# Dzh-16/FLASH-Viterbi

Hardware: AMD Instinct MI355X
Metric: trellis_cells_per_sec (higher is better)
Workload: dtype f32 scores (+f64 add per cell, rounded to f32 as the reference does)

## Files before the change

### flash_viterbi_amd/csrc/fv_context.hip

```cpp
#include "fv_internal.h"
#include "flashvit_testing.h"

namespace {

template <typename F>
void parallel_rows(int rows, F &&fn)
{
    unsigned hw = std::thread::hardware_concurrency();
    int nt = (int)std::min<unsigned>(hw ? hw : 4, 16);
    if (rows < 256) nt = 1;
    if (nt <= 1) { fn(0, rows); return; }
    std::vector<std::thread> th;
    int per = (rows + nt - 1) / nt;
    for (int t = 0; t < nt; ++t) {
        int a = t * per, b = std::min(rows, a + per);
        if (a >= b) break;
        th.emplace_back([=, &fn] { fn(a, b); });
    }
    for (auto &x : th) x.join();
}

}

namespace fvi {
// ... 922 lines not shown
        if (int rc = fvi::launch_stage_emissions(ctx, dev_scores, dtype, ld, T, ctx->EMap.p, ctx->emis_P, ctx->E32.p, ctx->E64.p, ctx->d_emflags.p)) return fvi::drained(ctx, rc);
    FV_HIP(hipEventRecord(e1, ctx->stream));
    FV_HIP(hipStreamSynchronize(ctx->stream));
    float ms = 0.0f;
    FV_HIP(hipEventElapsedTime(&ms, e0, e1));
    *ms_out = ms / (float)reps;
    ctx->stats.device_bytes = (long long)fvi::device_bytes(ctx);
    return FV_OK;
}

extern "C" int fv_test_flat_poison(fv_ctx *ctx, int t)
{
    if (!ctx || t < -1) return FV_ERR_ARG;
    FV_NO_STREAM(ctx);
    ctx->flat_poison = t;
    return FV_OK;
}

extern "C" int fv_set_option(fv_ctx *ctx, int key, long long value)
{
    if (!ctx) return FV_ERR_ARG;
    FV_NO_STREAM(ctx);
    if (ctx->group && ctx->group_rank == 0) {
        for (int r = fvi::group_size(ctx) - 1; r >= 1; --r) {
            const int rc = fv_set_option(fvi::group_member(ctx, r), key, value);
            if (rc) return rc;
        }
    }
    switch (key) {
    case FV_OPT_KERNEL:
        if ((value < FV_KERNEL_AUTO || value > FV_KERNEL_U16_REFINE) && value != FV_KERNEL_CSR_F64) return FV_ERR_ARG;
        ctx->opt_kernel = (int)value; return FV_OK;
    case FV_OPT_MAX_BATCH:
        if (value < 1 || value > fvk::MAX_BATCH) return FV_ERR_ARG;
        ctx->opt_max_batch = (int)value; return FV_OK;
    case FV_OPT_PROFILE:
        ctx->opt_profile = value ? 1 : 0; return FV_OK;
    case FV_OPT_FLAT_GENERATIONS:
        if (value < 0 || value > 2) return FV_ERR_ARG;
        ctx->opt_flat = (int)value; return FV_OK;
    case FV_OPT_ROW_CODES:
        if (value < 0 || value > 4) return FV_ERR_ARG;
        ctx->opt_row_codes = (int)value; return FV_OK;
    case FV_OPT_SEL_MARGIN:
        if (value < 0 || value > 100000) return FV_ERR_ARG;
        ctx->opt_sel_margin = (float)value * 1e-3f; return FV_OK;
    case FV_OPT_SPARSE_BEAM:
        if (value != 0 && value != 1) return FV_ERR_ARG;
        ctx->opt_sparse_beam = (int)value; return FV_OK;
    case FV_OPT_DEBUG:
#ifndef FV_TIMING_BUILD
        if (value & FV_DEBUG_TIMING_ONLY) { ctx->detail = "FV_OPT_DEBUG: result-changing timing switches need the timing build"; return FV_ERR_ARG; }
#endif
        if (value < 0 || value >= (1ll << 32) || (value & ((1ll << 27) | (1ll << 30)))) return FV_ERR_ARG;
        ctx->opt_csr_mem = (int)((value >> 31) & 1);
        ctx->opt_debug = (int)(value & 0x3fffffff); return FV_OK;
    default: return FV_ERR_ARG;
    }
}

extern "C" long long fv_checkpoint_memory_bytes(int K, int T, int step)
{
    if (step <= 0) step = (int)std::floor(std::sqrt(1.0 * T));
    const long long nck = (T + step - 1) / step;
    const long long last = T - (nck - 1) * step;
    const long long tsub = nck > 1 && step + 1 > last ? step + 1 : last;
    return 4LL * K + 4LL * K * nck + 4LL * K + 4LL * (T / step + 1) + 8LL * K * tsub;
}

extern "C" int fv_last_stats(const fv_ctx *ctx, fv_stats *out)
{
    if (!ctx || !out) return FV_ERR_ARG;
    *out = ctx->stats;
    return FV_OK;
}

extern "C" const char *fv_last_error_detail(const fv_ctx *ctx) { return ctx ? ctx->detail.c_str() : ""; }

extern "C" const char *fv_strerror(int rc)
{
    switch (rc) {
    case FV_OK: return "ok";
    case FV_WARN_BEAM_MISS: return "beam miss: path holds -1 entries, as the reference prints";
    case FV_ERR_ARG: return "bad argument";
    case FV_ERR_NOMEM: return "out of memory";
    case FV_ERR_NO_PRED: return "decoded entry has no finite predecessor";
    case FV_ERR_DEVICE: return "HIP error";
    case FV_ERR_STATE: return "call out of order (no model / no communicator)";
    case FV_ERR_UNSUPPORTED: return "size or option not supported by this build";
    case FV_ERR_COMM: return "RCCL error";
    default: return "unknown flashvit error";
    }
}

extern "C" long long fv_reference_memory_bytes(int K, int T, int n_split, int beam_width)
{
    const long long N = n_split;
    const long long pool = ((40 + 48 + 8 * N + 12 + 7) / 8) * 8;
    long long mem = 0, tmp;
    const bool nway = N > 2 && T >= 2 * N;
    if (beam_width <= 0) {
        if (nway) mem = 4 * (N - 1) + 2LL * K * 4 + 2 * (N - 1) * (long long)K * 4;
        tmp = N * (2LL * K * 4 + 2LL * K * 4);
    } else {
        if (nway) mem = 4 * (N - 1) + 2 * (N - 1) * (long long)(beam_width + 1) * 12;
        tmp = N * (2LL * (beam_width + 1) * 12);
    }
    if (tmp > mem) mem = tmp;
// ... 3 lines not shown
```

### flash_viterbi_amd/csrc/fv_full.hip

```cpp
#include "fv_internal.h"
#include "fv_kernels.hip.inc"
#include "flashvit_testing.h"

namespace {

int pick_kernel(const fv_ctx *ctx)
{
    if (ctx->opt_kernel == FV_KERNEL_F64_STREAM) return FV_KERNEL_F64_STREAM;
    if (!ctx->view.logs_nonpositive) return FV_KERNEL_F64_STREAM;
    if (ctx->opt_kernel == FV_KERNEL_F16_REFINE || ctx->opt_kernel == FV_KERNEL_F32_REFINE ||
        ctx->opt_kernel == FV_KERNEL_Q16_REFINE || ctx->opt_kernel == FV_KERNEL_U16_REFINE)
        return ctx->opt_kernel;
    if (ctx->opt_kernel == FV_KERNEL_SPARSE_Q16) return ctx->SPdata.p ? FV_KERNEL_SPARSE_Q16 : FV_KERNEL_U16_REFINE;
    return (ctx->SPdata.p && ctx->density <= 0.35) ? FV_KERNEL_SPARSE_Q16 : FV_KERNEL_U16_REFINE;
}

constexpr int U_UP = 16, U_DB32 = 4, U_DB64 = 2, U_DB16 = 2;

constexpr int nb_slot(int NB) { return NB == 1 ? 0 : NB == 2 ? 1 : NB == 4 ? 2 : 3; }
template <typename TA> constexpr int tab_slot()
{
    return std::is_same<TA, double>::value ? 0 : std::is_same<TA, float>::value ? 1 : std::is_same<TA, fvk::half_t>::value ? 2 : 3;
}
template <typename TA, int NB, bool DB> constexpr unsigned long long step_variant()
// ... 134 lines not shown
    a.data = ctx->SPdata.p; a.tile_off = ctx->SPoff.p; a.tile_nwb = ctx->SPnwb.p;
    a.LA64 = ctx->LA64.p; a.counters = ctx->d_counters.p;
    a.debug = ctx->opt_debug;
    a.window = ctx->windowq; a.qscale = ctx->qscale;
    if (ctx->test_record) ctx->test_variants |= sparse_variant<NB>();
    hipLaunchKernelGGL((fvk::trellis_step_sparse<NB>), dim3(a.tiles_per_xcd * 8), dim3(fvk::SP_BLOCK),
                       fvk::sparse_lds_bytes<NB>(ctx->nrows), ln.stream, a);
    FV_HIP(hipGetLastError());
    return 0;
}

template <typename Go>
void launch_csr_form(const fv_ctx *ctx, size_t lds_form_bytes, Go &&go)
{
    if (ctx->opt_csr_mem || lds_form_bytes > (size_t)fvk::LDS_LIMIT) go(std::true_type{});
    else go(std::false_type{});
}

template <int NB>
int launch_csr_nb(fv_ctx *ctx, const StepLaunch &ln, const fvk::TaskSlot *slots, int nb)
{
    fvk::CsrArgs<NB> a;
    fill_common(ctx, slots, nb, a);
    a.ck = ctx->CSk.p; a.cq = ctx->CSq.p; a.c64 = ctx->CS64.p; a.tile_off = ctx->CSoff.p; a.tile_nwb = ctx->CSnwb.p;
    a.counters = ctx->d_counters.p;
    a.debug = ctx->opt_debug;
    a.window = ctx->windowq; a.qscale = ctx->qscale;
    launch_csr_form(ctx, fvk::csr_lds_bytes<NB>(ctx->nrows, false), [&](auto MEM) {
        if (ctx->test_record) ctx->test_variants |= csr_variant<NB, MEM()>();
        hipLaunchKernelGGL((fvk::trellis_step_csr<NB, MEM()>), dim3(a.tiles_per_xcd * 8), dim3(fvk::SP_BLOCK),
                           fvk::csr_lds_bytes<NB>(ctx->nrows, MEM()), ln.stream, a);
    });
    FV_HIP(hipGetLastError());
    return 0;
}

template <int NB>
int launch_csr_f64_nb(fv_ctx *ctx, const StepLaunch &ln, const fvk::TaskSlot *slots, int nb)
{
    fvk::CsrF64Args<NB> a;
    fill_common(ctx, slots, nb, a);
    a.ck = ctx->CSk.p; a.c64 = ctx->CS64.p; a.tile_off = ctx->CSoff.p; a.tile_nwb = ctx->CSnwb.p;
    a.vanilla = ctx->vanilla;
    launch_csr_form(ctx, fvk::csr_f64_lds_bytes<NB>(ctx->nrows, false), [&](auto MEM) {
        if (ctx->test_record) ctx->test_variants |= csr_f64_variant<NB, MEM()>();
        hipLaunchKernelGGL((fvk::trellis_step_csr_f64<NB, MEM()>), dim3(a.tiles_per_xcd * 8), dim3(fvk::SP_BLOCK),
                           fvk::csr_f64_lds_bytes<NB>(ctx->nrows, MEM()), ln.stream, a);
    });
    FV_HIP(hipGetLastError());
    return 0;
}

template <int NB> constexpr bool U16_CODE_FREE = NB == 1;

template <int NB, int U, bool DB, int NWV>
int launch_u16_variant(fv_ctx *ctx, const StepLaunch &ln, const fvk::StepArgs<NB> &a)
{
    const size_t lds = fvk::u16_lds_bytes<NB, NWV>(ctx->nrows);
    fvk::StepArgs<NB> b = a;
    if (!fvk::u16_takes_codes<NB, DB, NWV>()) b.codes &= ~1;
    if (ctx->test_record) ctx->test_variants |= u16_variant<NB, DB, NWV>() | ((b.codes & 1) ? FV_TV_ROW_CODES : 0ull);
    if (U16_CODE_FREE<NB> && a.codes == 0)
        hipLaunchKernelGGL((fvk::trellis_step_u16<NB, U, DB, NWV, !U16_CODE_FREE<NB>>), dim3(a.tiles_per_xcd * 8), dim3(NWV * 64), lds, ln.stream, b);
    else
        hipLaunchKernelGGL((fvk::trellis_step_u16<NB, U, DB, NWV>), dim3(a.tiles_per_xcd * 8), dim3(NWV * 64), lds, ln.stream, b);
    FV_HIP(hipGetLastError());
    return 0;
}

template <int NB>
int launch_u16_nb(fv_ctx *ctx, const StepLaunch &ln, const LaunchCodes &lc, const fvk::TaskSlot *slots, int nb)
{
    fvk::StepArgs<NB> a;
    fill_step_args(ctx, ln, slots, nb, a);
    a.LA = ctx->LAQ16.p; a.window = ctx->windowq; a.vanilla = 0;
    a.codes = lc.codes;
    for (int t = 0; t < NB; ++t) a.c[t] = lc.slots[t < nb ? t : 0];
    const int nq = ctx->nrows / 32;
    if (ctx->opt_debug & 8192) {
        if (a.ntiles <= ctx->num_cus && (nq + 15) / 16 <= 8 && !(ctx->opt_debug & 4)) return launch_u16_variant<NB, 8, false, 16>(ctx, ln, a);
        return launch_u16_variant<NB, U_DB16, true, 16>(ctx, ln, a);
    }
    if (a.ntiles <= ctx->num_cus && (nq + 7) / 8 <= 16 && !(ctx->opt_debug & 4) && !ln.forked) return launch_u16_variant<NB, 16, false, 8>(ctx, ln, a);
    return launch_u16_variant<NB, U_DB16, true, 8>(ctx, ln, a);
}

constexpr int ROW_CODES_AUTO_MIN_K = 2048;
constexpr int ROW_CODES_AUTO_FAMILIES = 2;

int coded_row_index(const fv_ctx *ctx, const float *row)
{
    if (!row || row < ctx->d_rows.p || row >= ctx->d_rows.p + ctx->d_rows.n) return -1;
    const size_t off = (size_t)(row - ctx->d_rows.p);
    if (off % (size_t)ctx->nrows) return -1;
    const size_t r = off / (size_t)ctx->nrows;
    return r < ctx->row_coded.size() ? (int)r : -1;
}

int ensure_row_codes(fv_ctx *ctx, size_t pairs)
{
    if (!ctx->row_codes) { ctx->row_coded.clear(); return 0; }
    const size_t rows = pairs * 2, want = rows * (size_t)ctx->nrows;
    if (want > ctx->d_rcodes.n || want / fvk::TILE_W > ctx->d_rtmax.n) {
        if (ctx->d_rcodes.ensure(want) != hipSuccess || ctx->d_rtmax.ensure(want / fvk::TILE_W) != hipSuccess) {
            (void)hipGetLastError();
            ctx->d_rcodes.release(); ctx->d_rtmax.release();
            ctx->row_codes = 0; ctx->row_coded.clear();
            return 0;
        }
        FV_HIP(hipMemsetAsync(ctx->d_rcodes.p, 0xff, ctx->d_rcodes.bytes(), ctx->stream));
        FV_HIP(hipMemsetAsync(ctx->d_rtmax.p, 0xff, ctx->d_rtmax.bytes(), ctx->stream));
    }
    ctx->row_coded.assign(ctx->d_rcodes.n / (size_t)ctx->nrows, 0);
    return 0;
}

bool init_rows_coded(fv_ctx *ctx, int base, int n)
{
    if (!ctx->row_codes || ctx->csr || (size_t)(base + n) * 2 > ctx->row_coded.size()) return false;
    for (int q = 0; q < n; ++q) ctx->row_coded[(size_t)(base + q) * 2] = 1;
    return true;
}

int launch_step_kernel(fv_ctx *ctx, const StepLaunch &ln, const fvk::TaskSlot *slots, int nb)
{
    fvk::CodeSlot cs[fvk::MAX_BATCH];
    const bool packed = ln.kernel == FV_KERNEL_U16_REFINE && (nb <= 1 || !ctx->full_ok || (ctx->opt_debug & 16384) || ln.forked);
    bool all_in = packed && ctx->row_codes != 0, all_out = all_in;
    int rout[fvk::MAX_BATCH];
    for (int q = 0; q < nb; ++q) {
        const int rin = coded_row_index(ctx, slots[q].t1_in);
        rout[q] = coded_row_index(ctx, slots[q].t1_out);
        const size_t ntp = (size_t)ctx->nrows / fvk::TILE_W;
        cs[q].c_in = rin >= 0 ? ctx->d_rcodes.p + (size_t)rin * ctx->nrows : nullptr;
        cs[q].tmax_in = rin >= 0 ? ctx->d_rtmax.p + (size_t)rin * ntp : nullptr;
        cs[q].c_out = rout[q] >= 0 ? ctx->d_rcodes.p + (size_t)rout[q] * ctx->nrows : nullptr;
// ... 357 lines not shown
            if (++c.s > bt.len) { ++c.b; c.s = 1; }
        }
    }
    for (int sid = 0; sid < nstreams; ++sid) {
        std::vector<int> ones;
        for (int i = 0; i < np; ++i) if (fp.passes[i].batch < 0 && fp.passes[i].stream == sid) ones.push_back(i);
        if (ones.empty()) continue;
        if (col_last) { const int rc = columns(ones, stream_of(ctx, sid)); if (rc) return rc; continue; }
        const size_t cap = (size_t)std::max(1, ctx->flat_key[2]);
        for (size_t base = 0; base < ones.size(); base += cap) {
            const int nb = (int)std::min(cap, ones.size() - base);
            fvk::TaskSlot slots[fvk::MAX_BATCH];
            for (int q = 0; q < nb; ++q) {
                const int i = ones[base + q];
                slots[q] = task_slot(ctx, row(i, 0), row(i, 1), fp.passes[i].R, arg_rows(fp.passes[i]));
            }
            if (int rc = queue_step(ctx, StepLaunch{ kernel, stream_of(ctx, sid), two, 1 }, slots, nb)) return rc;
        }
    }
    if (int rc = join_streams(ctx, nstreams)) return rc;
    hipLaunchKernelGGL(fvk::backtrack_flat, dim3(np), dim3(64), 0, ctx->stream, ctx->d_flat.p, ctx->d_bp.p, ctx->d_flat_bp.p, K,
                       ctx->d_snap.p, ctx->d_chain.p, ctx->d_counters.p + fvk::BT_COUNTER);
    FV_HIP(hipGetLastError());
    fvk::FlatGens gens;
    gens.ngen = (int)fp.gen_begin.size() - 1;
    for (int g = 0; g <= gens.ngen; ++g) gens.begin[g] = fp.gen_begin[(size_t)g];
    hipLaunchKernelGGL(fvk::flat_resolve, dim3(1), dim3(1024), 0, ctx->stream, ctx->d_flat.p, gens, ctx->d_snap.p, ctx->d_chain.p,
                       ctx->d_ans.p, ctx->d_counters.p + fvk::FLAT_COUNTER);
    FV_HIP(hipGetLastError());
    ctx->stats.passes += np;
    ctx->stats.flat_passes = np;
    return 0;
}

}

namespace fvi {

template <int NB>
int setup_nb(fv_ctx *ctx)
{
    int rc = 0;
    if ((rc = allow_big_lds<float, NB>(ctx)) || (rc = allow_big_lds<double, NB>(ctx)) || (rc = allow_big_lds<fvk::half_t, NB>(ctx)) ||
        (rc = allow_big_lds<fvk::q16_t, NB>(ctx)) || (rc = set_big_lds(ctx, &fvk::trellis_step_sparse<NB>)) ||
        (rc = set_big_lds(ctx, &fvk::trellis_step_csr<NB, false>)) || (rc = set_big_lds(ctx, &fvk::trellis_step_csr_f64<NB, false>)) ||
        (rc = set_big_lds(ctx, &fvk::trellis_step_u16<NB, 8, false, 16>)) || (rc = set_big_lds(ctx, &fvk::trellis_step_u16<NB, U_DB16, true, 16>)) ||
        (rc = set_big_lds(ctx, &fvk::trellis_step_u16<NB, 16, false, 8>)) || (rc = set_big_lds(ctx, &fvk::trellis_step_u16<NB, U_DB16, true, 8>)))
        return rc;
    if constexpr (U16_CODE_FREE<NB>) {
        if ((rc = set_big_lds(ctx, &fvk::trellis_step_u16<NB, 8, false, 16, false>)) || (rc = set_big_lds(ctx, &fvk::trellis_step_u16<NB, U_DB16, true, 16, false>)) ||
            (rc = set_big_lds(ctx, &fvk::trellis_step_u16<NB, 16, false, 8, false>)) || (rc = set_big_lds(ctx, &fvk::trellis_step_u16<NB, U_DB16, true, 8, false>)))
            return rc;
    }
    return 0;
}

template <int... NB>
int setup_all(fv_ctx *ctx, NbList<NB...>)
{
    int rc = 0;
    (void)(((rc = setup_nb<NB>(ctx)) != 0) || ...);
    return rc;
}

int full_setup(fv_ctx *ctx) { return setup_all(ctx, STEP_NB); }

int launch_init_rows(fv_ctx *ctx, const fvk::PassChunk &ch, float *rows)
{
    return launch_init(ctx, ch, ctx->d_ans.p, rows, ctx->view.lb64, ctx->d_ob.p, false);
}

template <typename TIN>
static void launch_stage_as(fv_ctx *ctx, const void *src, long long ld, int T, const int *map, dim3 grid, float *E32, double *E64,
                            unsigned long long *flags)
{
    if (map)
        hipLaunchKernelGGL((fvk::stage_emissions<TIN, true>), grid, dim3(fvk::EMIS_BLOCK), 0, ctx->stream,
                           static_cast<const TIN *>(src), ld, T, ctx->K, map, E32, E64, flags);
    else
        hipLaunchKernelGGL((fvk::stage_emissions<TIN, false>), grid, dim3(fvk::EMIS_BLOCK), 0, ctx->stream,
                           static_cast<const TIN *>(src), ld, T, ctx->K, map, E32, E64, flags);
}

int launch_stage_emissions(fv_ctx *ctx, const void *src, int dtype, long long ld, int T, const int *map, int P,
                           float *E32, double *E64, unsigned long long *flags)
{
    const int K = ctx->K;
    const int gx = std::min((K + fvk::EMIS_BLOCK - 1) / fvk::EMIS_BLOCK, 2048), gy = std::max(1, std::min(T, 2048 / gx));
    if (P <= 0) map = nullptr;
    switch (dtype) {
    case FV_EMIS_LOG_F64: launch_stage_as<double>(ctx, src, ld, T, map, dim3(gx, gy), E32, E64, flags); break;
    case FV_EMIS_LOG_F32: launch_stage_as<float>(ctx, src, ld, T, map, dim3(gx, gy), E32, E64, flags); break;
    case FV_EMIS_LOG_F16: launch_stage_as<_Float16>(ctx, src, ld, T, map, dim3(gx, gy), E32, E64, flags); break;
    case FV_EMIS_LOG_BF16: launch_stage_as<fvk::bf16_bits>(ctx, src, ld, T, map, dim3(gx, gy), E32, E64, flags); break;
    default: ctx->detail = "fv_set_emissions: unknown dtype"; return FV_ERR_ARG;
    }
    FV_HIP(hipGetLastError());
    return 0;
}


int stream_init_row(fv_ctx *ctx, const double *lb64, const int *sym, float *row)
{
    fvk::PassChunk ch;
    ch.n = 1;
    ch.p[0] = fvk::PassDesc{ 0, 0, 1, 1, 0 };
// ... 407 lines not shown
```

### flash_viterbi_amd/csrc/fv_internal.h

```cpp
#pragma once

#include <hip/hip_runtime.h>
#include <rccl/rccl.h>

#include <algorithm>
#include <chrono>
#include <condition_variable>
#include <functional>
#include <mutex>
#include <cmath>
#include <cstdio>
#include <cstdlib>
#include <cstring>
#include <string>
#include <thread>
#include <vector>

#include "flashvit.h"
#include "fv_layout.h"
#include "fv_schedule.h"

using clk = std::chrono::steady_clock;
inline double ms_since(clk::time_point t0) { return std::chrono::duration<double, std::milli>(clk::now() - t0).count(); }

// ... 63 lines not shown
    struct EmisView {
        const float *lb32 = nullptr;
        const double *lb64 = nullptr;
        int nsym = 0;
        bool logs_nonpositive = false;
    } view;

    DevBuf<int> d_ob, d_ans, d_bp, d_gather;
    DevBuf<float> d_rows, d_score, d_ckpt;
    DevBuf<unsigned long long> d_counters;
    DevBuf<unsigned short> d_rcodes;
    DevBuf<float> d_rtmax;
    std::vector<unsigned char> row_coded;
    int row_codes = 0;
    DevBuf<int> d_snap, d_flat_bp, d_chain;
    DevBuf<fvk::FlatDesc> d_flat;
    fv::FlatPlan flat_plan;
    int flat_key[4] = { 0, 0, 0, 0 };
    const void *flat_uploaded = nullptr;
    int flat_poison = -1;
    DevBuf<int> d_pack;
    int *h_pin = nullptr;
    size_t h_pin_n = 0;
    DevBuf<float> d_hval, d_scores, d_slot_val;
    DevBuf<int> d_hstate, d_slot_state, d_flags;
    DevBuf<double> LA64R;
    DevBuf<unsigned short> LAQ16R;
    bool rowq_ready = false, beam_q16_ready = false;
    DevBuf<unsigned long long> d_qaux;
    DevBuf<int2> d_tie_list;
    DevBuf<float> d_cut;
    DevBuf<fvb::HNode> d_cand;
    DevBuf<int> d_cand_count;
    float opt_sel_margin = 0.3f;
    DevBuf<int> d_dupwin;
    DevBuf<int> d_doubt, d_doubt_count;
    DevBuf<int> d_needfull;
    DevBuf<int> d_seqof;
    std::vector<int> h_seqof;
    DevBuf<int> d_passL;
    std::vector<int> h_passL;
    DevBuf<unsigned int> d_tie_count;
    DevBuf<unsigned long long> d_csr_acc;
    DevBuf<unsigned int> d_csr_tie;
    long long csr_nnz = 0;

    int opt_sparse_beam = 0;
    int opt_kernel = FV_KERNEL_AUTO;
    int opt_max_batch = fvk::MAX_BATCH;
    int opt_profile = 0;
    int opt_flat = 1;
    int opt_row_codes = 1;
    int vanilla = 0;
    int opt_csr_mem = 0;
    int opt_debug = 0;
    std::vector<hipEvent_t> prof_events;
    std::vector<int> h_ob;
    std::vector<hipGraphExec_t> graphs;
    bool test_record = false;
    unsigned long long test_variants = 0;
    unsigned long long test_selects = 0;

    ncclComm_t comm = nullptr;
    int rank = 0, nranks = 1;
    struct fv_group *group = nullptr;
    int group_rank = 0;

    struct fv_stream *strm = nullptr;
    fv_stream_stats strm_stats{};
    bool strm_any = false;

    fv_stats stats{};
    void start_stats(int kernel, int generations, long long table_bytes_per_step, double density_reported)
    {
        const double model_ms = stats.set_model_ms, emis_ms = stats.set_emissions_ms;
        const long long rows = stats.emission_rows;
        stats = fv_stats{};
        stats.set_model_ms = model_ms; stats.set_emissions_ms = emis_ms; stats.emission_rows = rows;
        stats.kernel = kernel; stats.generations = generations;
        stats.table_bytes_per_step = table_bytes_per_step; stats.density = density_reported;
        stats.flat_first_miss = -1;
    }
    void close_stats(long long cells_per_task_step, long long cells_per_column_step)
    {
        stats.cells = stats.task_steps * cells_per_task_step + stats.column_steps * cells_per_column_step;
        stats.alg_bytes = 4 * stats.cells;
    }

    template <class F>
    void each_buffer(F &&f) const
    {
        f(LA32); f(LB32T); f(LA16); f(LAQ16); f(SPdata); f(SPoff); f(SPnwb); f(LA64); f(LB64T); f(LPi64);
        f(CSk); f(CSq); f(CS64); f(CSoff); f(CSnwb); f(CRptr); f(CRcol); f(CRlog);
        f(E32); f(E64); f(d_emflags); f(EMap);
        f(d_ob); f(d_ans); f(d_bp); f(d_gather); f(d_rows); f(d_rcodes); f(d_rtmax); f(d_score); f(d_ckpt); f(d_counters); f(d_pack);
        f(d_snap); f(d_flat_bp); f(d_chain); f(d_flat);
        f(d_hval); f(d_scores); f(d_slot_val); f(d_hstate); f(d_slot_state); f(d_flags); f(LA64R); f(LAQ16R); f(d_qaux);
        f(d_tie_list); f(d_cut); f(d_cand); f(d_cand_count); f(d_dupwin); f(d_doubt); f(d_doubt_count); f(d_needfull);
        f(d_seqof); f(d_passL); f(d_tie_count); f(d_csr_acc); f(d_csr_tie);
    }
};

#define FV_HIP(call)                                                                          \
    do {                                                                                      \
        hipError_t e_ = (call);                                                               \
        if (e_ != hipSuccess) {                                                               \
// ... 108 lines not shown
```

### flash_viterbi_amd/csrc/fv_kernels.hip.inc

```
#pragma once

#include <hip/hip_runtime.h>

#include <cfloat>
#include <climits>
#include <cstdint>
#include <type_traits>

#include "fv_device_common.h"

#ifdef FV_TIMING_BUILD
#define FV_TIMING_BIT(debug, bit) (((debug) & (bit)) != 0)
#else
#define FV_TIMING_BIT(debug, bit) false
#endif

namespace fvk {


struct TaskSlot {
    const float *t1_in;
    float *t1_out;
    int *bp_out;
    const float *tmp_row;
// ... 436 lines not shown
#pragma unroll
    for (int t = 0; t < NB; ++t) {
        float r = rr[t];
        int kb = rk[t];
        wave_best(r, kb);
        if (lane < TILE_W) { redR[(t * TILE_W + c) * NWV + w] = r; redK[(t * TILE_W + c) * NWV + w] = kb; }
    }
    __syncthreads();
    if (w < NB && w < args.nb) {
        const float4 fv = *reinterpret_cast<const float4 *>(redR + (w * TILE_W + c) * NWV + (rg * 4) % NWV);
        const int4 fk = *reinterpret_cast<const int4 *>(redK + (w * TILE_W + c) * NWV + (rg * 4) % NWV);
        float r = fv.x;
        int kb = fk.x;
        if (better(fv.y, fk.y, r, kb)) { r = fv.y; kb = fk.y; }
        if (better(fv.z, fk.z, r, kb)) { r = fv.z; kb = fk.z; }
        if (better(fv.w, fk.w, r, kb)) { r = fv.w; kb = fk.w; }
        wave_best(r, kb);
        if (lane < TILE_W && col < K) {
            if (args.merge) {
                const float pv = args.t[w].t1_out[col];
                const int pk = args.t[w].bp_out[col];
                if (pk >= 0 && !(r > pv)) { r = pv; kb = pk; }
            }
            const bool any = r > -FLT_MAX;
            args.t[w].t1_out[col] = any ? r : -FLT_MAX;
            args.t[w].bp_out[col] = any ? kb : -1;
        }
    }
}


typedef unsigned short fv_u16x2 __attribute__((ext_vector_type(2)));
__device__ __forceinline__ unsigned int pk_adds(unsigned int a, unsigned int b)
{
    return __builtin_bit_cast(unsigned int, __builtin_elementwise_add_sat(__builtin_bit_cast(fv_u16x2, a), __builtin_bit_cast(fv_u16x2, b)));
}
__device__ __forceinline__ unsigned int pk_minu(unsigned int a, unsigned int b)
{
    return __builtin_bit_cast(unsigned int, __builtin_elementwise_min(__builtin_bit_cast(fv_u16x2, a), __builtin_bit_cast(fv_u16x2, b)));
}
__device__ __forceinline__ unsigned int pk_maxu(unsigned int a, unsigned int b)
{
    return __builtin_bit_cast(unsigned int, __builtin_elementwise_max(__builtin_bit_cast(fv_u16x2, a), __builtin_bit_cast(fv_u16x2, b)));
}

__device__ __forceinline__ unsigned int score_code(float mx, float v, float inv_step)
{
    const float q = (mx - v) * inv_step;
    return (v > -0.5f * FLT_MAX && q < 65534.5f) ? (unsigned int)__float2uint_rn(q) : 65535u;
}

template <int NB, bool DB, int NWV> constexpr bool u16_takes_codes() { return !(NB == 8 && NWV == 16 && !DB); }

template <int NB, int U, bool DB, int NWV, bool CODES = true>
__global__ __launch_bounds__(NWV * 64) void trellis_step_u16(const StepArgs<NB> args)
{
    constexpr int R = 8, RBR = 32;
    extern __shared__ __align__(16) unsigned char smem[];
    const int nrows = args.nrows, npairs = nrows >> 1;
    unsigned int *T1c = reinterpret_cast<unsigned int *>(smem);
    unsigned int *redZ = T1c + (size_t)NB * npairs;
    float *redR = reinterpret_cast<float *>(redZ + NB * NWV * TILE_W);
    int *redK = reinterpret_cast<int *>(redR + NB * NWV * TILE_W);
    unsigned int *colZ = reinterpret_cast<unsigned int *>(redK + NB * NWV * TILE_W);

    const int tid = threadIdx.x, lane = tid & 63, w = tid >> 6;
    const int c = lane & (TILE_W - 1), rg = lane >> 4;
    const int tile = (blockIdx.x & 7) * args.tiles_per_xcd + (blockIdx.x >> 3);
    if (tile >= args.ntiles) return;
    const int col = tile * TILE_W + c;
    const int K = args.K;
    const bool rev = args.reverse != 0;
    const unsigned short *tile_base = reinterpret_cast<const unsigned short *>(args.LA) + (size_t)tile * nrows * TILE_W;
    const uint4 *LAt = reinterpret_cast<const uint4 *>(tile_base) + rg * TILE_W + c;
    const int nq = nrows / RBR;
    const int nj = nq > w ? (nq - w + NWV - 1) / NWV : 0;
    auto block_of = [&](int p) { return w + NWV * (rev ? nj - 1 - p : p); };

    float Mx[NB], tmp[NB];
    const float step = -args.qscale, inv_step = 1.0f / step;
    const int nq4 = nrows >> 2;
    constexpr int QPT = 1024 / (NWV * 64);
    uint4 cur[U], nxt[DB ? U : 1];
    auto request_table = [&]() {
        __builtin_amdgcn_sched_barrier(0);
#pragma unroll
        for (int u = 0; u < U; ++u)
            if (u < nj) cur[u] = LAt[(size_t)block_of(u) * (4 * TILE_W)];
        __builtin_amdgcn_sched_barrier(0);
#pragma unroll
        for (int t = 0; t < NB; ++t) tmp[t] = args.t[t].tmp_row[min(col, K - 1)];
        __builtin_amdgcn_sched_barrier(0);
    };
    const bool coded = CODES && u16_takes_codes<NB, DB, NWV>() && (args.codes & 1) != 0;
    const int nch = nrows >> 3;
    if (coded) {
        uint4 cv[NB];
        float tw[NB], tm[NB][4];
        const int ch = min(tid, nch - 1);
#pragma unroll
        for (int t = 0; t < NB; ++t) cv[t] = reinterpret_cast<const uint4 *>(args.c[t].c_in)[ch];
        auto request_maxima = [&]() {
#pragma unroll
            for (int t = 0; t < NB; ++t) {
                tw[t] = args.c[t].tmax_in[ch >> 1];
#pragma unroll
                for (int j = 0; j < 4; ++j) tm[t][j] = args.c[t].tmax_in[min(lane + 64 * j, args.ntiles - 1)];
            }
        };
        if constexpr (NB < 8) request_maxima();
        request_table();
        if constexpr (NB >= 8) request_maxima();
#pragma unroll
        for (int t = 0; t < NB; ++t) {
            float x = fmaxf(fmaxf(tm[t][0], tm[t][1]), fmaxf(tm[t][2], tm[t][3]));
            for (int i = 256 + lane; i < args.ntiles; i += 64) x = fmaxf(x, args.c[t].tmax_in[i]);
#pragma unroll
// ... 125 lines not shown
        m2[t] = min(max(lo, hi), min(m2p[t] & 0xffffu, m2p[t] >> 16));
    }

    constexpr bool SPEC = !DB && NB <= 2;
    double Lc[NB];
    float tv[NB];
    const double *L64t = args.LA64 + (size_t)tile * nrows * TILE_W + c * 4;
    const int blk0 = nj > 0 ? block_of(0) : 0;
    auto locate = [&](int t, int blk, const uint4 &ce, unsigned int &second) -> int {
        const unsigned int ca[4] = { ce.x, ce.y, ce.z, ce.w };
        const uint4 ct4 = *reinterpret_cast<const uint4 *>(T1c + (size_t)t * npairs + blk * (RBR / 2) + rg * (R / 2));
        const unsigned int ct[4] = { ct4.x, ct4.y, ct4.z, ct4.w };
        const int k0 = blk * RBR + rg * R;
        int found = k0 + par[t];
        unsigned int b1 = 0xffffffffu, b2 = 0xffffffffu;
#pragma unroll
        for (int i = 3; i >= 0; --i) {
            const unsigned int z = pk_adds(ca[i], ct[i]);
            b2 = pk_minu(b2, pk_maxu(z, b1));
            b1 = pk_minu(b1, z);
            const unsigned int zh = par[t] ? (z >> 16) : (z & 0xffffu);
            found = zh == m1[t] ? k0 + 2 * i + par[t] : found;
        }
        second = par[t] ? (b2 >> 16) : (b2 & 0xffffu);
        return found;
    };
    if constexpr (SPEC) {
#pragma unroll
        for (int t = 0; t < NB; ++t) {
            const int blk = a1[t] >= 0 ? a1[t] : blk0;
            const int jj = (blk - w) / NWV;
            const int pos = rev ? nj - 1 - jj : jj;
            uint4 ce = cur[0];
#pragma unroll
            for (int u = 1; u < U; ++u) {
                const bool hit = u == pos;
                ce.x = hit ? cur[u].x : ce.x; ce.y = hit ? cur[u].y : ce.y; ce.z = hit ? cur[u].z : ce.z; ce.w = hit ? cur[u].w : ce.w;
            }
            unsigned int second;
            const int found = locate(t, blk, ce, second);
            m2[t] = a1[t] >= 0 ? min(m2[t], second) : m2[t];
            a1[t] = a1[t] >= 0 ? found : -1;
        }
    }

    unsigned int Zc[NB];
#pragma unroll
    for (int t = 0; t < NB; ++t) {
        unsigned int v = m1[t];
        v = min(v, (unsigned int)__shfl_xor((int)v, 16));
        v = min(v, (unsigned int)__shfl_xor((int)v, 32));
        if (lane < TILE_W) redZ[(t * TILE_W + c) * NWV + w] = v;
    }
    __syncthreads();
    if constexpr (NB <= 2) {
#pragma unroll
        for (int t = 0; t < NB; ++t) {
            const uint4 *q = reinterpret_cast<const uint4 *>(redZ + (t * TILE_W + c) * NWV);
            unsigned int v = 0xffffffffu;
#pragma unroll
            for (int x = 0; x < NWV / 4; ++x) {
                const uint4 f = q[x];
                v = min(min(v, min(f.x, f.y)), min(f.z, f.w));
            }
            Zc[t] = v;
        }
    } else {
        if (w < NB) {
            const uint4 f = *reinterpret_cast<const uint4 *>(redZ + (w * TILE_W + c) * NWV + (rg * 4) % NWV);
            unsigned int v = min(min(f.x, f.y), min(f.z, f.w));
            v = min(v, (unsigned int)__shfl_xor((int)v, 16));
            v = min(v, (unsigned int)__shfl_xor((int)v, 32));
            if (lane < TILE_W) colZ[w * TILE_W + c] = v;
        }
        __syncthreads();
#pragma unroll
        for (int t = 0; t < NB; ++t) Zc[t] = colZ[t * TILE_W + c];
    }

    float rr[NB];
    int rk[NB];
    {
        int kind[NB];
        unsigned int thrs[NB];
#pragma unroll
        for (int t = 0; t < NB; ++t) {
            kind[t] = 0;
            thrs[t] = 0;
            if (t < args.nb && col < K && !FV_TIMING_BIT(args.debug, 4096)) {
                const float zz = fabsf(Mx[t] + tmp[t]) + 65536.0f * step + 1.0f;
                const unsigned int eb = __float_as_uint(zz) & 0x7f800000u;
                const float Uf = (eb > (24u << 23) && eb < 0x7f800000u) ? __uint_as_float(eb - (23u << 23)) : (eb >= 0x7f800000u ? 0.0f : FLT_MIN);
                const float wf = (2.0f * Uf + args.window) * inv_step + (coded ? 4.2f : 3.1f);
                const unsigned int W = wf < 65535.0f ? (unsigned int)wf + 1u : 65535u;
                const unsigned int thr = Zc[t] + W;
                thrs[t] = thr;
                if (thr >= 65535u) {
                    kind[t] = 2;
                    if (w == 0 && rg == 0) atomicAdd(&args.counters[8], 1ull);
                }
                else if (m2[t] <= thr) kind[t] = 2;
                else if (m1[t] <= thr && a1[t] >= 0) kind[t] = 1;
            }
        }
        if constexpr (SPEC) {
#pragma unroll
            for (int t = 0; t < NB; ++t) {
                Lc[t] = 0.0; tv[t] = 0.0f;
                if (kind[t] == 1) {
                    Lc[t] = L64t[(size_t)(a1[t] >> 2) * (TILE_W * 4) + (a1[t] & 3)];
                    tv[t] = args.t[t].t1_in[a1[t]];
                }
            }
        } else {
            uint4 ce[NB];
#pragma unroll
            for (int t = 0; t < NB; ++t) ce[t] = LAt[(size_t)(kind[t] == 1 ? a1[t] : blk0) * (4 * TILE_W)];
#pragma unroll
            for (int t = 0; t < NB; ++t) {
                unsigned int second;
                const int found = locate(t, kind[t] == 1 ? a1[t] : blk0, ce[t], second);
                kind[t] = (kind[t] == 1 && second <= thrs[t]) ? 2 : kind[t];
                a1[t] = found;
                Lc[t] = L64t[(size_t)(found >> 2) * (TILE_W * 4) + (found & 3)];
                tv[t] = args.t[t].t1_in[found];
            }
        }
#pragma unroll
        for (int t = 0; t < NB; ++t) {
            float r = FV_NEG_INF;
            int kb = INT_MAX;
            if (kind[t] == 1) {
                r = exact_cell(tmp[t], tv[t], Lc[t]);
                kb = a1[t];
                if (m1[t] != Zc[t]) atomicAdd(&args.counters[0], 1ull);
            }
            rr[t] = r; rk[t] = kb;
        }
        const double *L64tile = args.LA64 + (size_t)tile * nrows * TILE_W;
#pragma unroll
        for (int t = 0; t < NB; ++t) {
            unsigned long long need = __ballot(kind[t] == 2);
            while (need) {
                const int L = __ffsll((long long)need) - 1;
                need &= need - 1;
                const int cL = L & (TILE_W - 1), rgL = L >> 4;
                const float tmpL = __shfl(tmp[t], L);
                const float *t1g = args.t[t].t1_in;
                float bx = FV_NEG_INF;
                int bk = INT_MAX;
                const int nlane_rows = nj * R;
                for (int e0 = 0; e0 < nlane_rows; e0 += 128) {
                    int kk[2];
                    float tt[2];
                    double LL[2];
#pragma unroll
                    for (int u = 0; u < 2; ++u) {
                        const int e = e0 + 64 * u + lane;
                        const int k = (w + NWV * (e / R)) * RBR + rgL * R + (e % R);
                        kk[u] = (e < nlane_rows && k < K) ? k : -1;
                        const int ks = kk[u] >= 0 ? k : 0;
                        tt[u] = t1g[ks];
                        LL[u] = L64tile[(size_t)(ks >> 2) * (TILE_W * 4) + cL * 4 + (ks & 3)];
                    }
#pragma unroll
                    for (int u = 0; u < 2; ++u) {
                        if (kk[u] >= 0) {
                            const float x = exact_cell(tmpL, tt[u], LL[u]);
                            if (better(x, kk[u], bx, bk)) { bx = x; bk = kk[u]; }
                        }
                    }
                }
#pragma unroll
                for (int m = 1; m < 64; m <<= 1) {
                    const float ov = __shfl_xor(bx, m);
                    const int ok = __shfl_xor(bk, m);
                    if (better(ov, ok, bx, bk)) { bx = ov; bk = ok; }
                }
                if (lane == L) { rr[t] = bx; rk[t] = bk; }
                if (lane == 0) atomicAdd(&args.counters[1], 1ull);
            }
        }
    }

#pragma unroll
    for (int t = 0; t < NB; ++t) {
        float r = rr[t];
        int kb = rk[t];
        wave_best(r, kb);
        if (lane < TILE_W) { redR[(t * TILE_W + c) * NWV + w] = r; redK[(t * TILE_W + c) * NWV + w] = kb; }
    }
    __syncthreads();
    if (w < NB && w < args.nb) {
        const float4 fv = *reinterpret_cast<const float4 *>(redR + (w * TILE_W + c) * NWV + (rg * 4) % NWV);
        const int4 fk = *reinterpret_cast<const int4 *>(redK + (w * TILE_W + c) * NWV + (rg * 4) % NWV);
        float r = fv.x;
        int kb = fk.x;
        if (better(fv.y, fk.y, r, kb)) { r = fv.y; kb = fk.y; }
        if (better(fv.z, fk.z, r, kb)) { r = fv.z; kb = fk.z; }
        if (better(fv.w, fk.w, r, kb)) { r = fv.w; kb = fk.w; }
        wave_best(r, kb);
        const bool any = r > -FLT_MAX;
        if (lane < TILE_W && col < K) {
            args.t[w].t1_out[col] = any ? r : -FLT_MAX;
            args.t[w].bp_out[col] = any ? kb : -1;
        }
        if (CODES && (args.codes & 2)) {
            const float val = (col < K && any) ? r : -FLT_MAX;
            float tmx = val;
#pragma unroll
            for (int m = 1; m < TILE_W; m <<= 1) tmx = fmaxf(tmx, __shfl_xor(tmx, m));
            if (lane < TILE_W) {
                args.c[w].c_out[col] = (unsigned short)score_code(tmx, val, inv_step);
                if (lane == 0) args.c[w].tmax_out[tile] = tmx;
            }
        }
    }
}

__global__ void q16_tile_range(const double *t4, size_t n, unsigned long long *lmax_bits)
{
    double m = 0.0;
    for (size_t e = (size_t)blockIdx.x * blockDim.x + threadIdx.x; e < n; e += (size_t)gridDim.x * blockDim.x) {
        const double l = t4[e];
        if (l > -__builtin_huge_val() && -l > m) m = -l;
    }
#pragma unroll
    for (int k = 1; k < 64; k <<= 1) { const double o = __shfl_xor(m, k); m = o > m ? o : m; }
    if ((threadIdx.x & 63) == 0 && m > 0.0) atomicMax(lmax_bits, (unsigned long long)__double_as_longlong(m));
}

__global__ void q16_tile_codes(const double *t4, unsigned short *q8, int K, int nrows, int ntiles,
                               const unsigned long long *lmax_bits, unsigned long long *dmax_bits)
{
    const double lmax = __longlong_as_double((long long)*lmax_bits);
    const float stepf = lmax > 0.0 ? (float)(lmax / 65534.0) : 1.0f;
    const double stepd = (double)stepf;
    const size_t n = (size_t)ntiles * nrows * TILE_W;
    double dm = 0.0;
    for (size_t e = (size_t)blockIdx.x * blockDim.x + threadIdx.x; e < n; e += (size_t)gridDim.x * blockDim.x) {
        const int tile = (int)(e / ((size_t)nrows * TILE_W));
        const int rem = (int)(e % ((size_t)nrows * TILE_W));
        const int k = rem / TILE_W, col = tile * TILE_W + rem % TILE_W;
        unsigned short code = 0xFFFFu;
        const double l = t4[tab_index<4>(k, col, nrows)];
        if (k < K && col < K && l > -__builtin_huge_val()) {
            double c = nearbyint(-l / stepd);
            c = c < 0.0 ? 0.0 : (c > 65534.0 ? 65534.0 : c);
            code = (unsigned short)c;
            const double d = fabs(-c * stepd - l);
            dm = d > dm ? d : dm;
        }
        q8[tab_index<8>(k, col, nrows)] = code;
    }
#pragma unroll
    for (int k = 1; k < 64; k <<= 1) { const double o = __shfl_xor(dm, k); dm = o > dm ? o : dm; }
    if ((threadIdx.x & 63) == 0 && dm > 0.0) atomicMax(dmax_bits, (unsigned long long)__double_as_longlong(dm));
}


constexpr int SP_WAVES = 8;
constexpr int SP_BLOCK = SP_WAVES * 64;

template <int NB>
struct SparseArgs {
    const uint4 *data;
    const int *tile_off;
    const int *tile_nwb;
    const double *LA64;
// ... 840 lines not shown
```

### flash_viterbi_amd/csrc/fv_layout.h

```cpp
#pragma once

#include <hip/hip_runtime.h>

#include <cstddef>

namespace fvk {

constexpr int TILE_W = 16;
constexpr int ROWG = 64 / TILE_W;
constexpr int NWAVES = 16;
constexpr int BLOCK = NWAVES * 64;
constexpr int ROW_ALIGN = 32;
constexpr int MAX_BATCH = 8;
constexpr int LDS_LIMIT = 160 * 1024;

template <int R>
__host__ __device__ inline size_t tab_index(int k, int col, int nrows)
{
    return (size_t)(col >> 4) * nrows * TILE_W + ((size_t)(k / R) * TILE_W + (col & 15)) * R + (k % R);
}
constexpr int BT_WARMUP = 32, BT_MIN_PARALLEL = 128;
struct PassDesc { int L, R, from_pi, whole; long long row_off; };
constexpr int PASS_CHUNK = 64;
struct PassChunk { int n; PassDesc p[PASS_CHUNK]; };
struct FlatDesc { int L, R, generation, chain; long long arg_row; };
constexpr int FLAT_MAX_GENS = 40;
struct FlatGens { int ngen; int begin[FLAT_MAX_GENS + 1]; };
constexpr int FLAT_COUNTER = 15;
constexpr int BT_COUNTER = 16;

template <int NB>
static inline size_t step_lds_bytes(int nrows)
{
    return (size_t)nrows * NB * 4 + (size_t)NB * NWAVES * TILE_W * 12 + (size_t)NB * TILE_W * 4;
}

template <int NB, int NWV>
static inline size_t u16_lds_bytes(int nrows)
{
    return (size_t)nrows * NB * 2 + (size_t)NB * NWV * TILE_W * 12 + (size_t)NB * TILE_W * 4;
}

}
```

Measured before the change: 1217 billion.

## Compact refine candidates into an LDS work list for batched u16 step

```diff
diff --git a/flash_viterbi_amd/csrc/fv_context.hip b/flash_viterbi_amd/csrc/fv_context.hip
--- a/flash_viterbi_amd/csrc/fv_context.hip
+++ b/flash_viterbi_amd/csrc/fv_context.hip
@@ -998,8 +998,9 @@
 #ifndef FV_TIMING_BUILD
         if (value & FV_DEBUG_TIMING_ONLY) { ctx->detail = "FV_OPT_DEBUG: result-changing timing switches need the timing build"; return FV_ERR_ARG; }
 #endif
-        if (value < 0 || value >= (1ll << 32) || (value & ((1ll << 27) | (1ll << 30)))) return FV_ERR_ARG;
+        if (value < 0 || value >= (1ll << 34) || (value & ((1ll << 27) | (1ll << 30) | (1ll << 32)))) return FV_ERR_ARG;
         ctx->opt_csr_mem = (int)((value >> 31) & 1);
+        ctx->opt_wave_tail = (int)((value >> 33) & 1);
         ctx->opt_debug = (int)(value & 0x3fffffff); return FV_OK;
     default: return FV_ERR_ARG;
     }
diff --git a/flash_viterbi_amd/csrc/fv_full.hip b/flash_viterbi_amd/csrc/fv_full.hip
--- a/flash_viterbi_amd/csrc/fv_full.hip
+++ b/flash_viterbi_amd/csrc/fv_full.hip
@@ -210,14 +210,20 @@
 }
 
 template <int NB> constexpr bool U16_CODE_FREE = NB == 1;
-
-template <int NB, int U, bool DB, int NWV>
+template <int NB> constexpr bool U16_LIST = NB >= 2;
+
+template <int NB, int U, bool DB, int NWV, bool LIST = false>
 int launch_u16_variant(fv_ctx *ctx, const StepLaunch &ln, const fvk::StepArgs<NB> &a)
 {
-    const size_t lds = fvk::u16_lds_bytes<NB, NWV>(ctx->nrows);
+    const size_t lds = LIST ? fvk::u16_list_lds_bytes<NB, NWV>(ctx->nrows) : fvk::u16_lds_bytes<NB, NWV>(ctx->nrows);
     fvk::StepArgs<NB> b = a;
     if (!fvk::u16_takes_codes<NB, DB, NWV>()) b.codes &= ~1;
     if (ctx->test_record) ctx->test_variants |= u16_variant<NB, DB, NWV>() | ((b.codes & 1) ? FV_TV_ROW_CODES : 0ull);
+    if constexpr (LIST) {
+        hipLaunchKernelGGL((fvk::trellis_step_u16<NB, U, DB, NWV, true, true>), dim3(a.tiles_per_xcd * 8), dim3(NWV * 64), lds, ln.stream, b);
+        FV_HIP(hipGetLastError());
+        return 0;
+    }
     if (U16_CODE_FREE<NB> && a.codes == 0)
         hipLaunchKernelGGL((fvk::trellis_step_u16<NB, U, DB, NWV, !U16_CODE_FREE<NB>>), dim3(a.tiles_per_xcd * 8), dim3(NWV * 64), lds, ln.stream, b);
     else
@@ -240,6 +246,13 @@
         return launch_u16_variant<NB, U_DB16, true, 16>(ctx, ln, a);
     }
     if (a.ntiles <= ctx->num_cus && (nq + 7) / 8 <= 16 && !(ctx->opt_debug & 4) && !ln.forked) return launch_u16_variant<NB, 16, false, 8>(ctx, ln, a);
+    if constexpr (U16_LIST<NB>) {
+        constexpr size_t BY_REGS = NB >= 8 ? 2 : NB >= 4 ? 3 : 4;
+        const size_t with = fvk::u16_list_lds_bytes<NB, 8>(ctx->nrows), without = fvk::u16_lds_bytes<NB, 8>(ctx->nrows);
+        if (!ctx->opt_wave_tail && with <= (size_t)fvk::LDS_LIMIT &&
+            std::min((size_t)fvk::LDS_LIMIT / with, BY_REGS) >= std::min((size_t)fvk::LDS_LIMIT / without, BY_REGS))
+            return launch_u16_variant<NB, U_DB16, true, 8, true>(ctx, ln, a);
+    }
     return launch_u16_variant<NB, U_DB16, true, 8>(ctx, ln, a);
 }
 
@@ -703,6 +716,9 @@
             (rc = set_big_lds(ctx, &fvk::trellis_step_u16<NB, 16, false, 8, false>)) || (rc = set_big_lds(ctx, &fvk::trellis_step_u16<NB, U_DB16, true, 8, false>)))
             return rc;
     }
+    if constexpr (U16_LIST<NB>) {
+        if ((rc = set_big_lds(ctx, &fvk::trellis_step_u16<NB, U_DB16, true, 8, true, true>))) return rc;
+    }
     return 0;
 }
 
diff --git a/flash_viterbi_amd/csrc/fv_internal.h b/flash_viterbi_amd/csrc/fv_internal.h
--- a/flash_viterbi_amd/csrc/fv_internal.h
+++ b/flash_viterbi_amd/csrc/fv_internal.h
@@ -139,6 +139,7 @@
     int opt_flat = 1;
     int opt_row_codes = 1;
     int vanilla = 0;
+    int opt_wave_tail = 0;
     int opt_csr_mem = 0;
     int opt_debug = 0;
     std::vector<hipEvent_t> prof_events;
diff --git a/flash_viterbi_amd/csrc/fv_kernels.hip.inc b/flash_viterbi_amd/csrc/fv_kernels.hip.inc
--- a/flash_viterbi_amd/csrc/fv_kernels.hip.inc
+++ b/flash_viterbi_amd/csrc/fv_kernels.hip.inc
@@ -512,9 +512,25 @@
 
 template <int NB, bool DB, int NWV> constexpr bool u16_takes_codes() { return !(NB == 8 && NWV == 16 && !DB); }
 
-template <int NB, int U, bool DB, int NWV, bool CODES = true>
+__device__ __forceinline__ unsigned long long refine_key(float v, int row)
+{
+    const unsigned int b = __float_as_uint(v);
+    const unsigned int neg0 = b == 0x80000000u ? 1u : 0u;
+    const unsigned int cb = neg0 ? 0u : b;
+    const unsigned int o = (cb & 0x80000000u) ? ~cb : (cb | 0x80000000u);
+    return ((unsigned long long)o << 32) | ((unsigned long long)(~(unsigned int)row & 0x7fffffffu) << 1) | neg0;
+}
+__device__ __forceinline__ float refine_key_value(unsigned long long key)
+{
+    const unsigned int o = (unsigned int)(key >> 32);
+    return __uint_as_float((key & 1ull) ? 0x80000000u : ((o & 0x80000000u) ? (o & 0x7fffffffu) : ~o));
+}
+__device__ __forceinline__ int refine_key_row(unsigned long long key) { return (int)(~(unsigned int)(key >> 1) & 0x7fffffffu); }
+
+template <int NB, int U, bool DB, int NWV, bool CODES = true, bool LIST = false>
 __global__ __launch_bounds__(NWV * 64) void trellis_step_u16(const StepArgs<NB> args)
 {
+    static_assert(!LIST || DB, "the list tail is built for the double-buffered forms");
     constexpr int R = 8, RBR = 32;
     extern __shared__ __align__(16) unsigned char smem[];
     const int nrows = args.nrows, npairs = nrows >> 1;
@@ -522,7 +538,13 @@
     unsigned int *redZ = T1c + (size_t)NB * npairs;
     float *redR = reinterpret_cast<float *>(redZ + NB * NWV * TILE_W);
     int *redK = reinterpret_cast<int *>(redR + NB * NWV * TILE_W);
-    unsigned int *colZ = reinterpret_cast<unsigned int *>(redK + NB * NWV * TILE_W);
+    constexpr int NLIST = 64 * NWV * NB;
+    unsigned long long *slot = reinterpret_cast<unsigned long long *>(redZ + NB * NWV * TILE_W);
+    unsigned int *colZ = LIST ? reinterpret_cast<unsigned int *>(slot + NB * TILE_W)
+                              : reinterpret_cast<unsigned int *>(redK + NB * NWV * TILE_W);
+    float *tmpS = reinterpret_cast<float *>(colZ + NB * TILE_W);
+    uint2 *list = reinterpret_cast<uint2 *>(tmpS + NB * TILE_W);
+    unsigned int *cnt = reinterpret_cast<unsigned int *>(list + NLIST);
 
     const int tid = threadIdx.x, lane = tid & 63, w = tid >> 6;
     const int c = lane & (TILE_W - 1), rg = lane >> 4;
@@ -754,6 +776,14 @@
         v = min(v, (unsigned int)__shfl_xor((int)v, 32));
         if (lane < TILE_W) redZ[(t * TILE_W + c) * NWV + w] = v;
     }
+    if constexpr (LIST) {
+        if (tid < NB * TILE_W) slot[tid] = 0ull;
+        if (tid < TILE_W) {
+#pragma unroll
+            for (int t = 0; t < NB; ++t) tmpS[t * TILE_W + c] = tmp[t];
+        }
+        if (tid == 0) *cnt = 0u;
+    }
     __syncthreads();
     if constexpr (NB <= 2) {
 #pragma unroll
@@ -780,11 +810,9 @@
         for (int t = 0; t < NB; ++t) Zc[t] = colZ[t * TILE_W + c];
     }
 
-    float rr[NB];
-    int rk[NB];
+    int kind[NB];
+    unsigned int thrs[NB];
     {
-        int kind[NB];
-        unsigned int thrs[NB];
 #pragma unroll
         for (int t = 0; t < NB; ++t) {
             kind[t] = 0;
@@ -805,6 +833,158 @@
                 else if (m1[t] <= thr && a1[t] >= 0) kind[t] = 1;
             }
         }
+    }
+
+    auto store_result = [&](float r, int kb) {
+        const bool any = r > -FLT_MAX;
+        if (lane < TILE_W && col < K) {
+            args.t[w].t1_out[col] = any ? r : -FLT_MAX;
+            args.t[w].bp_out[col] = any ? kb : -1;
+        }
+        if (CODES && (args.codes & 2)) {
+            const float val = (col < K && any) ? r : -FLT_MAX;
+            float tmx = val;
+#pragma unroll
+            for (int m = 1; m < TILE_W; m <<= 1) tmx = fmaxf(tmx, __shfl_xor(tmx, m));
+            if (lane < TILE_W) {
+                args.c[w].c_out[col] = (unsigned short)score_code(tmx, val, inv_step);
+                if (lane == 0) args.c[w].tmax_out[tile] = tmx;
+            }
+        }
+    };
+
+    if constexpr (LIST) {
+        const double *L64tile = args.LA64 + (size_t)tile * nrows * TILE_W;
+        auto t1_of = [&](int tt) {
+            const float *p = args.t[0].t1_in;
+#pragma unroll
+            for (int t = 1; t < NB; ++t) p = tt == t ? args.t[t].t1_in : p;
+            return p;
+        };
+        auto submit = [&](int tt, int cc, float r, int k) {
+            if (r > -FLT_MAX) atomicMax(&slot[tt * TILE_W + cc], refine_key(r, k));
+        };
+        auto rewalk = [&](int ow, int rgL, int cL, int tt) {
+            const float tmpL = tmpS[tt * TILE_W + cL];
+            const float *t1g = t1_of(tt);
+            float bx = FV_NEG_INF;
+            int bk = INT_MAX;
+            const int nlane_rows = (nq > ow ? (nq - ow + NWV - 1) / NWV : 0) * R;
+            for (int e0 = 0; e0 < nlane_rows; e0 += 128) {
+                int kk[2];
+                float tt2[2];
+                double LL[2];
+#pragma unroll
+                for (int u = 0; u < 2; ++u) {
+                    const int e = e0 + 64 * u + lane;
+                    const int k = (ow + NWV * (e / R)) * RBR + rgL * R + (e % R);
+                    kk[u] = (e < nlane_rows && k < K) ? k : -1;
+                    const int ks = kk[u] >= 0 ? k : 0;
+                    tt2[u] = t1g[ks];
+                    LL[u] = L64tile[(size_t)(ks >> 2) * (TILE_W * 4) + cL * 4 + (ks & 3)];
+                }
+#pragma unroll
+                for (int u = 0; u < 2; ++u) {
+                    if (kk[u] >= 0) {
+                        const float x = exact_cell(tmpL, tt2[u], LL[u]);
+                        if (better(x, kk[u], bx, bk)) { bx = x; bk = kk[u]; }
+                    }
+                }
+            }
+#pragma unroll
+            for (int m = 1; m < 64; m <<= 1) {
+                const float ov = __shfl_xor(bx, m);
+                const int ok = __shfl_xor(bk, m);
+                if (better(ov, ok, bx, bk)) { bx = ov; bk = ok; }
+            }
+            if (lane == 0) {
+                submit(tt, cL, bx, bk);
+                atomicAdd(&args.counters[1], 1ull);
+            }
+        };
+
+        unsigned long long b1[NB], b2[NB];
+        unsigned int tot = 0;
+#pragma unroll
+        for (int t = 0; t < NB; ++t) {
+            b1[t] = __ballot(kind[t] == 1);
+            b2[t] = __ballot(kind[t] == 2);
+            tot += (unsigned int)__popcll(b1[t]) + ((unsigned int)__popcll(b2[t]) << 16);
+        }
+        if (tot) {
+            unsigned int base = 0;
+            if (lane == 0) base = atomicAdd(cnt, tot);
+            base = (unsigned int)__shfl((int)base, 0);
+            unsigned int s0 = base & 0xffffu, j0 = base >> 16;
+#pragma unroll
+            for (int t = 0; t < NB; ++t) {
+                if (kind[t] == 1) {
+                    const unsigned int pos = s0 + __builtin_amdgcn_mbcnt_hi((unsigned int)(b1[t] >> 32), __builtin_amdgcn_mbcnt_lo((unsigned int)b1[t], 0u));
+                    list[pos] = make_uint2((unsigned int)tid | ((unsigned int)t << 10) | ((unsigned int)par[t] << 13) |
+                                           (m1[t] != Zc[t] ? 1u << 14 : 0u) | ((unsigned int)a1[t] << 16), m1[t] | (thrs[t] << 16));
+                } else if (kind[t] == 2) {
+                    const unsigned int pos = j0 + __builtin_amdgcn_mbcnt_hi((unsigned int)(b2[t] >> 32), __builtin_amdgcn_mbcnt_lo((unsigned int)b2[t], 0u));
+                    list[NLIST - 1 - pos] = make_uint2((unsigned int)tid | ((unsigned int)t << 10), 0u);
+                }
+                s0 += (unsigned int)__popcll(b1[t]);
+                j0 += (unsigned int)__popcll(b2[t]);
+            }
+        }
+        __syncthreads();
+
+        const unsigned int counts = *cnt;
+        const unsigned int nsingle = counts & 0xffffu, njob = counts >> 16;
+        for (unsigned int e0 = (unsigned int)w * 64u; e0 < nsingle; e0 += NWV * 64u) {
+            const bool valid = e0 + lane < nsingle;
+            const uint2 en = list[valid ? e0 + lane : e0];
+            const int oc = en.x & (TILE_W - 1), org = (en.x >> 4) & 3, tt = (en.x >> 10) & 7, opar = (en.x >> 13) & 1, blk = (int)(en.x >> 16);
+            const unsigned int om1 = en.y & 0xffffu, othr = en.y >> 16;
+            const uint4 ce = reinterpret_cast<const uint4 *>(tile_base)[(size_t)blk * (4 * TILE_W) + org * TILE_W + oc];
+            const unsigned int ca[4] = { ce.x, ce.y, ce.z, ce.w };
+            const uint4 ct4 = *reinterpret_cast<const uint4 *>(T1c + (size_t)tt * npairs + blk * (RBR / 2) + org * (R / 2));
+            const unsigned int ct[4] = { ct4.x, ct4.y, ct4.z, ct4.w };
+            const int k0 = blk * RBR + org * R;
+            int found = k0 + opar;
+            unsigned int q1 = 0xffffffffu, q2 = 0xffffffffu;
+#pragma unroll
+            for (int i = 3; i >= 0; --i) {
+                const unsigned int z = pk_adds(ca[i], ct[i]);
+                q2 = pk_minu(q2, pk_maxu(z, q1));
+                q1 = pk_minu(q1, z);
+                const unsigned int zh = opar ? (z >> 16) : (z & 0xffffu);
+                found = zh == om1 ? k0 + 2 * i + opar : found;
+            }
+            const unsigned int second = opar ? (q2 >> 16) : (q2 & 0xffffu);
+            const bool promoted = valid && second <= othr;
+            const double Lx = L64tile[(size_t)(found >> 2) * (TILE_W * 4) + oc * 4 + (found & 3)];
+            const float tx = t1_of(tt)[found];
+            if (valid && !promoted) {
+                submit(tt, oc, exact_cell(tmpS[tt * TILE_W + oc], tx, Lx), found);
+                if (en.x & (1u << 14)) atomicAdd(&args.counters[0], 1ull);
+            }
+            unsigned long long need = __ballot(promoted);
+            while (need) {
+                const int L = __ffsll((long long)need) - 1;
+                need &= need - 1;
+                const unsigned int x = (unsigned int)__shfl((int)en.x, L);
+                rewalk((x >> 6) & 15, (x >> 4) & 3, x & (TILE_W - 1), (x >> 10) & 7);
+            }
+        }
+        for (unsigned int j = (unsigned int)w; j < njob; j += NWV) {
+            const unsigned int x = (unsigned int)__builtin_amdgcn_readfirstlane((int)list[NLIST - 1 - j].x);
+            rewalk((x >> 6) & 15, (x >> 4) & 3, x & (TILE_W - 1), (x >> 10) & 7);
+        }
+        __syncthreads();
+        if (w < NB && w < args.nb) {
+            const unsigned long long key = slot[w * TILE_W + c];
+            store_result(key ? refine_key_value(key) : FV_NEG_INF, key ? refine_key_row(key) : INT_MAX);
+        }
+        return;
+    }
+
+    float rr[NB];
+    int rk[NB];
+    {
         if constexpr (SPEC) {
 #pragma unroll
             for (int t = 0; t < NB; ++t) {
@@ -902,21 +1082,7 @@
         if (better(fv.z, fk.z, r, kb)) { r = fv.z; kb = fk.z; }
         if (better(fv.w, fk.w, r, kb)) { r = fv.w; kb = fk.w; }
         wave_best(r, kb);
-        const bool any = r > -FLT_MAX;
-        if (lane < TILE_W && col < K) {
-            args.t[w].t1_out[col] = any ? r : -FLT_MAX;
-            args.t[w].bp_out[col] = any ? kb : -1;
-        }
-        if (CODES && (args.codes & 2)) {
-            const float val = (col < K && any) ? r : -FLT_MAX;
-            float tmx = val;
-#pragma unroll
-            for (int m = 1; m < TILE_W; m <<= 1) tmx = fmaxf(tmx, __shfl_xor(tmx, m));
-            if (lane < TILE_W) {
-                args.c[w].c_out[col] = (unsigned short)score_code(tmx, val, inv_step);
-                if (lane == 0) args.c[w].tmax_out[tile] = tmx;
-            }
-        }
+        store_result(r, kb);
     }
 }
 
diff --git a/flash_viterbi_amd/csrc/fv_layout.h b/flash_viterbi_amd/csrc/fv_layout.h
--- a/flash_viterbi_amd/csrc/fv_layout.h
+++ b/flash_viterbi_amd/csrc/fv_layout.h
@@ -41,4 +41,10 @@
     return (size_t)nrows * NB * 2 + (size_t)NB * NWV * TILE_W * 12 + (size_t)NB * TILE_W * 4;
 }
 
+template <int NB, int NWV>
+static inline size_t u16_list_lds_bytes(int nrows)
+{
+    return (size_t)nrows * NB * 2 + (size_t)NB * NWV * TILE_W * 4 + (size_t)NB * TILE_W * 16 + (size_t)64 * NWV * NB * 8 + 16;
 }
+
+}
```

Result: faster. 1243 billion, median of 6 (+2.1%).
